# huakunyang/SummerTTS

Hardware: AMD Instinct MI355X
Metric: audio samples/sec (acoustic model + vocoder, phoneme ids -> int16 PCM on host), single_speaker_fast-shaped synthetic blob (higher is better)
Workload: dtype f32 (decoder trunk convs AND the reverse flow's WaveNet convs (wn_flow.hip, one-utterance calls): fp32 operands as 2 fp16 terms = 22-23 of their 24 mantissa bits, 3 fp16 MFMA products per fp32 product, f32 accumulation -- measured error in `parity`, same tolerance as the exact-fp32 leg; batches addi

## Files before the change

### include/summertts_hip.h

```cpp
#ifndef SUMMERTTS_HIP_H_
#define SUMMERTTS_HIP_H_

#include <stdint.h>

#ifdef __cplusplus
extern "C" {
#endif

typedef struct sts_engine sts_engine;

enum {
    STS_OK = 0,
    STS_EINVAL = -1,
    STS_EMODEL = -2,
    STS_EDEVICE = -3,
    STS_ESTATE = -4
};

int sts_create(const float* blob, int64_t blob_bytes, int device, sts_engine** out);
void sts_destroy(sts_engine* e);

int sts_speaker_num(const sts_engine* e);

typedef struct sts_model_info {
// ... 144 lines not shown

enum { STS_DBG_ATTN_BLOCK_MIN_WGS = 1,
       STS_DBG_TAIL_FUSED = 14 ,
       STS_DBG_UPS_ROWPH = 15 ,
       STS_DBG_CHAIN_STREAMS = 13 ,
       STS_DBG_H2P = 11 ,
       STS_DBG_H2P_TILE = 12 ,
       STS_DBG_MEMO_CLEAR = 10 ,
       STS_DBG_PCM_DIRECT = 9 ,
       STS_DBG_DDS_TAIL = 8 ,
       STS_DBG_ATTN_REG = 7 ,
       STS_DBG_LAUNCH_AHEAD = 6 ,
       STS_DBG_FLOW_FUSED = 5  };
enum { STS_DBG_STREAM_RETRY_STEP = 16, STS_DBG_STREAM_DIRECT = 17 };
enum { STS_DBG_POISON = 18 };
int sts_debug_set(sts_engine* e, int key, int value);

typedef struct sts_profile {
    float ms_text_encoder, ms_duration, ms_flow, ms_decoder, ms_total_device;
    float ms_decoder_mfma;
    int32_t decoder_mfma_launches;
    double flops_text_encoder, flops_duration, flops_flow, flops_decoder;
    double flops_decoder_mfma;
    double bytes_decoder_min;
    int64_t frames, samples, phonemes;
    double flops_decoder_mfma_executed;
    double bytes_text_encoder, bytes_duration, bytes_flow;
    float ms_sync_wait_host;
    double flops_decoder_bf16_issued;
    int64_t conv_math_fallbacks;
// ... 115 lines not shown
```

### summertts_amd/csrc/capi.hip

```cpp
#include <stdlib.h>
#include <string.h>

#include <algorithm>
#include <new>
#include <string>
#include <utility>
#include <vector>

#include "engine.hpp"
#include "eq_stream.hpp"
#include "join_stream.hpp"
#include "loud_stream.hpp"

using namespace sts;

struct sts_engine { Engine eng; };

static thread_local std::string g_err;
static int set_err(int code, const std::string& s) { g_err = s; return code; }
#define STS_CAPI_NOT_WHILE_OPEN(e) \
    do { if ((e)->eng.stream_is_open()) return set_err(STS_ESTATE, "a stream is open on this engine (sts_stream_close first)"); } while (0)

extern "C" {

// ... 726 lines not shown
        case STS_DBG_ATTN_BLOCK_MIN_WGS: if (value < 1) return set_err(STS_EINVAL, "threshold must be >= 1"); e->eng.attn_block_min_wgs = value; return STS_OK;
        case STS_DBG_FLOW_FUSED: e->eng.flow_fused = value == 2 || value == 3 ? value : value != 0; return STS_OK;
        case STS_DBG_LAUNCH_AHEAD: if (value < 0 || value > 2) return set_err(STS_EINVAL, "launch_ahead must be 0, 1 or 2"); if ((value == 2) != (e->eng.launch_ahead == 2)) { e->eng.seen_tf_.clear(); e->eng.seen_order_.clear(); } e->eng.launch_ahead = value; return STS_OK;
        case STS_DBG_H2P: e->eng.h2p = value < 0 ? 0 : (value > 4 ? 4 : value); return STS_OK;
        case STS_DBG_H2P_TILE: e->eng.h2p_tile = value; return STS_OK;
        case STS_DBG_CHAIN_STREAMS: e->eng.chain_streams_dbg = value; return STS_OK;
        case STS_DBG_TAIL_FUSED: e->eng.tail_fused = value != 0; return STS_OK;
        case STS_DBG_UPS_ROWPH: e->eng.ups_rowph = value != 0; return STS_OK;
        case STS_DBG_MEMO_CLEAR: e->eng.seen_tf_.clear(); e->eng.seen_order_.clear(); return STS_OK;
        case STS_DBG_ATTN_REG: e->eng.attn_reg = value != 0; return STS_OK;
        case STS_DBG_DDS_TAIL: e->eng.dds_tail = value != 0; return STS_OK;
        case STS_DBG_PCM_DIRECT: e->eng.pcm_direct = value != 0; return STS_OK;
        case STS_DBG_STREAM_RETRY_STEP: e->eng.stream_retry_step = value < 0 ? -1 : value; return STS_OK;
        case STS_DBG_STREAM_DIRECT: e->eng.stream_direct = value != 0; return STS_OK;
        case STS_DBG_POISON: e->eng.poison = (unsigned)value; return STS_OK;
        default: return set_err(STS_EINVAL, "unknown debug key");
    }
}
int sts_set_host_pcm(sts_engine* e, int enable) { if (!e) return set_err(STS_EINVAL, "null engine"); e->eng.host_pcm = enable != 0; return STS_OK; }
int sts_set_profiling(sts_engine* e, int enable) { if (!e) return set_err(STS_EINVAL, "null engine"); e->eng.profiling = enable == 2 ? 2 : (enable != 0 ? 1 : 0); return STS_OK; }

int sts_abi_version(void) { return STS_ABI_VERSION; }

int sts_set_output_rate(sts_engine* e, int32_t rate) {
    if (!e) return set_err(STS_EINVAL, "null engine");
    const int rc = e->eng.set_output_rate(rate);
    return rc == STS_OK ? STS_OK : set_err(rc, e->eng.error());
}
int sts_get_output_rate(const sts_engine* e) {
    if (!e) return set_err(STS_EINVAL, "null engine");
// ... 835 lines not shown
```

### summertts_amd/csrc/conv.hip

```cpp
#include "kernels.hpp"
#include "devmath.hpp"
#include "conv_common.hpp"

namespace sts {

__device__ __forceinline__ float load_in(const ConvArgs& a, const float* xrow, int pos, int in_len, int orig_len) {
    if (pos < 0 || pos >= in_len) return 0.f;
    int src = pos;
    if (a.in_reflect) {
        src = pos - 1;
        if (src < 0) { if (orig_len > 1) src = 1; else return 0.f; }
    }
    float v = xrow[src];
    if (a.in_act) v = v < 0.f ? v * a.in_slope : v;
    return v;
}

#ifndef STS_EXP
#define STS_EXP 0
#endif

#ifndef STS_RA_GROUP
#define STS_RA_GROUP 3
#endif
// ... 769 lines not shown
            }
            static_for<0, 8>([&](auto rc) {
                constexpr int r = decltype(rc)::value;
                const int row = m0 + ((hb + r) & 3) + 8 * ((hb + r) >> 2) + 4 * half;
                const float bv = b2v[r];
                const float ya = acc[0][hb + r] + acc[1][hb + r] + acc[2][hb + r] + bv;
                const float yb = acc[1][hb + r] - acc[2][hb + r] - acc[3][hb + r] + bv;
                const size_t o = (size_t)row * G.ld + opos;
                if (va) a.y[o] = ya + xa[r];
                if (vb) a.y[o + 1] = yb + xb[r];
            });
        });
    }
}

template <int MW, int NW>
__global__ __launch_bounds__(1024) void conv_mfma_splitk_kernel(ConvArgs a, int mtiles) {
    constexpr int G = 4, E = MW * NW * 16;
    constexpr int D = MW * NW == 1 ? 6 : (MW * NW == 2 ? 4 : 3);
    extern __shared__ __attribute__((aligned(16))) float red[];
    const int KS = blockDim.x >> 6;
    const int nsl = a.kslices > 1 ? a.kslices : 1;
    const int b = blockIdx.z / nsl, slice = blockIdx.z - b * nsl;
    const int orig_len = seg_len(a.in_seg, b);
    const int in_len = orig_len + (a.in_reflect ? 1 : 0);
    const int out_len = seg_len(a.out_seg, b);
    const int n_count = a.transposed ? in_len + a.n_extra : out_len;
    const int n0 = blockIdx.x * 32 * NW;
    if (n0 >= n_count) return;
    const int phase = blockIdx.y / mtiles;
    const int m0 = (blockIdx.y - phase * mtiles) * 32 * MW;
    const size_t in_base = (size_t)seg_start(a.in_seg, b), out_base = (size_t)seg_start(a.out_seg, b);
    const int tid = threadIdx.x, lane = tid & 63, wave = tid >> 6;
    const int l31 = lane & 31, half = lane >> 5;
    const float* w = a.w + (size_t)phase * a.ntap * a.Cin_pad * a.Cout_pad;
    bool mvalid[MW];
#pragma unroll
    for (int i = 0; i < MW; i++) mvalid[i] = (m0 + i * 32) < a.Cout_pad;

    f32x16 acc[MW][NW];
#pragma unroll
    for (int i = 0; i < MW; i++)
#pragma unroll
        for (int q = 0; q < NW; q++)
#pragma unroll
            for (int r = 0; r < 16; r++) acc[i][q][r] = 0.f;

    const int gpt = a.Cin_pad / (2 * G);
    const int gall = a.ntap * gpt;
    const int gper = (gall + nsl - 1) / nsl;
    const int gfirst = slice * gper;
    const int ngroups = (STS_EXP & 64) ? gfirst : (gfirst + gper < gall ? gfirst + gper : gall);
    float ra[D][G][MW], rb[D][G][NW];
    const int swave = __builtin_amdgcn_readfirstlane(wave);
    const int sKS = __builtin_amdgcn_readfirstlane(KS);
    const rsrc_t xrs = make_rsrc(a.x + in_base, (unsigned)(((size_t)(a.Cin - 1) * a.x_ld + orig_len) * 4));
    const rsrc_t wrs = make_rsrc(w, (unsigned)((size_t)a.ntap * a.Cin_pad * a.Cout_pad * 4));
    const unsigned ld4 = (unsigned)a.x_ld * 4u;
    const unsigned x_lane = (unsigned)half * ld4;
    const unsigned a_lane = (unsigned)(((size_t)half * a.Cout_pad + m0 + l31) * 4);
    const int lanepos = n0 + l31;
    int lj = (gfirst + swave) / gpt, lc = (gfirst + swave - lj * gpt) * 2 * G;
    const int jstep = sKS / gpt, cstep = (sKS - jstep * gpt) * 2 * G;

    auto load_group = [&](float (&fa)[G][MW], float (&fb)[G][NW]) {
        const int shift = lj * a.tap_step + a.tap_off;
        unsigned off[NW];
#pragma unroll
        for (int q = 0; q < NW; q++) {
            int pos = lanepos + q * 32 + shift;
            bool v = pos >= 0 && pos < in_len;
            if (a.in_reflect) { pos = pos - 1; if (pos < 0) { pos = 1; v = v && orig_len > 1; } }
            off[q] = v ? (unsigned)pos * 4u + x_lane : kOOB;
        }
        const unsigned xs0 = (unsigned)lc * ld4;
        const unsigned ws0 = (unsigned)((((size_t)lj * a.Cin_pad + lc) * a.Cout_pad) * 4);
#pragma unroll
        for (int i = 0; i < G; i++) {
            const bool cv = lc + 2 * i + half < a.Cin;
#pragma unroll
            for (int q = 0; q < NW; q++)
                fb[i][q] = __builtin_bit_cast(float, __builtin_amdgcn_raw_buffer_load_b32(xrs, (int)(cv ? off[q] : kOOB), (int)(xs0 + (unsigned)(2 * i) * ld4), 0));
#pragma unroll
            for (int k = 0; k < MW; k++)
                fa[i][k] = __builtin_bit_cast(float, __builtin_amdgcn_raw_buffer_load_b32(
                    wrs, (int)a_lane, (int)(ws0 + (unsigned)(2 * i) * (unsigned)a.Cout_pad * 4u + (unsigned)k * 128u), 0));
        }
        lj += jstep; lc += cstep;
        if (lc >= a.Cin_pad) { lc -= a.Cin_pad; lj++; }
    };

    int gnext = gfirst + swave;
#pragma unroll
    for (int d = 0; d < D; d++) { if (gnext < ngroups) load_group(ra[d], rb[d]); gnext += sKS; }
    int gcur = gfirst + swave;
    while (gcur < ngroups) {
#pragma unroll
        for (int d = 0; d < D; d++) {
            if (gcur < ngroups) {
#pragma unroll
                for (int i = 0; i < G; i++) {
                    float bq[NW];
#pragma unroll
                    for (int q = 0; q < NW; q++) {
                        float v = rb[d][i][q];
                        if (a.in_act) v = v < 0.f ? v * a.in_slope : v;
                        bq[q] = v;
                    }
#pragma unroll
                    for (int k = 0; k < MW; k++)
#pragma unroll
                        for (int q = 0; q < NW; q++)
                            acc[k][q] = __builtin_amdgcn_mfma_f32_32x32x2f32(ra[d][i][k], bq[q], acc[k][q], 0, 0, 0);
                }
                if (gnext < ngroups) load_group(ra[d], rb[d]);
            }
            gnext += sKS; gcur += sKS;
        }
    }

    static_for<0, MW>([&](auto ic) {
        constexpr int i = decltype(ic)::value;
        static_for<0, NW>([&](auto qc) {
            constexpr int q = decltype(qc)::value;
            static_for<0, 16>([&](auto rc) {
                constexpr int r = decltype(rc)::value;
                red[((size_t)wave * E + (i * NW + q) * 16 + r) * 64 + lane] = acc[i][q][r];
            });
        });
    });
    __syncthreads();
    const int out_off = a.out_off + phase;
    const bool gate = a.epi == EPI_GATE;
    for (int e = wave; e < E; e += KS) {
        const int i = e / (NW * 16);
        const int q = (e >> 4) % NW, r = e & 15;
        if (gate && r >= 8) continue;
        const int n = n0 + q * 32 + l31;
        const int pos = n * a.out_stride + out_off;
        if (n >= n_count || pos < 0 || pos >= out_len) continue;
        const size_t opos = out_base + (size_t)pos;
        const int rowp = m0 + i * 32 + (r & 3) + 8 * (r >> 2) + 4 * half;
        float v = 0.f, v2 = 0.f;
        for (int k = 0; k < KS; k++) {
            v += red[((size_t)k * E + (i * NW + q) * 16 + r) * 64 + lane];
            if (gate) v2 += red[((size_t)k * E + (i * NW + q) * 16 + r + 8) * 64 + lane];
        }
        if (gate) {
            if (!mvalid[i]) continue;
// ... 43 lines not shown
    const long nt = (a.max_n + 127) / 128;
    if (a.Cout_pad % 64 == 0 && nt * (a.Cout_pad / 64) * nphase * a.B >= 512) return 3;
    return 4;
}

template <int MW, int NW, int WM, int WN>
static void launch_mfma(const ConvArgs& a, int nphase, hipStream_t st) {
    constexpr int MT = 32 * MW * WM, NT = 32 * NW * WN;
    const int mt = (a.Cout_pad + MT - 1) / MT;
    const int nx = (a.max_n + NT - 1) / NT, ny = mt * nphase;
    size_t lds = (size_t)2 * CK * (NT + MAX_HALO) * sizeof(float);
    hipLaunchKernelGGL((conv_mfma_kernel<MW, NW, WM, WN>), dim3(mapped_grid(nx, ny, a.B)), dim3(WM * WN * 64), lds, st, a, mt, nx, ny);
}

template <int MW, int NW>
static void launch_splitk(const ConvArgs& a, int nphase, hipStream_t st, bool pinned = false) {
    const int mt = (a.Cout_pad + 32 * MW - 1) / (32 * MW);
    const int nt = (a.max_n + 32 * NW - 1) / (32 * NW);
    const int nsl = a.kslices > 1 ? a.kslices : 1;
    const long steps = ((long)a.ntap * (a.Cin_pad / 8) + nsl - 1) / nsl;
    constexpr int E = MW * NW * 16;
    const bool sparse = !pinned && (long)mt * nt * nphase * a.B * nsl <= 256;
    const int ks_cap = E <= 16 ? 16 : (E <= 32 ? (sparse ? 16 : 8) : 4);
    int ks = 1;
    while (ks < ks_cap && steps / (ks * 2) >= 6 && (pinned || (long)mt * nt * nphase * a.B * nsl * ks * 2 <= 4096)) ks *= 2;
    dim3 grid(nt, mt * nphase, a.B * nsl);
    size_t lds = (size_t)ks * E * 64 * sizeof(float);
    hipLaunchKernelGGL((conv_mfma_splitk_kernel<MW, NW>), grid, dim3(ks * 64), lds, st, a, mt);
}

template <int MW, int NW, int WM, int WN>
static void launch_mfma_group(const ConvGroup& G, hipStream_t st) {
    constexpr int MT = 32 * MW * WM, NT = 32 * NW * WN;
    const ConvArgs& a = G.g[0];
    const int mt = (a.Cout_pad + MT - 1) / MT;
    const int nx = (a.max_n + NT - 1) / NT;
    size_t lds = (size_t)2 * CK * (NT + MAX_HALO) * sizeof(float);
    hipLaunchKernelGGL((conv_mfma_group_kernel<MW, NW, WM, WN>), dim3(mapped_grid(nx, mt, a.B * G.n)), dim3(WM * WN * 64), lds, st, G,
                       mt, a.B, nx, mt);
}

bool resblock_layer_eligible(const ResLayerGroup& G) {
    if (G.n < 1 || G.n > kMaxGroup || (G.C != 32 && G.C != 64 && G.C != 128) || G.max_n <= 0 || G.B <= 0) return false;
// ... 113 lines not shown
            ConvArgs t = G.g[j]; G.g[j] = G.g[j - 1]; G.g[j - 1] = t;
        }
    if (tile != 1 && tile != 3 && tile != 4 && tile != 5) {
        const ConvArgs& a = G.g[0];
        const long nt = (a.max_n + 127) / 128;
        tile = (a.Cout_pad % 64 == 0 && nt * (a.Cout_pad / 64) * a.B * G.n >= 1024) ? 3 : 4;
    }
    switch (tile) {
        case 1: launch_mfma_group<2, 2, 1, 4>(G, st); break;
        case 3: launch_mfma_group<2, 1, 1, 4>(G, st); break;
        case 5: launch_mfma_group<1, 2, 1, 4>(G, st); break;
        default: launch_mfma_group<1, 1, 1, 4>(G, st); break;
    }
}

void conv_mfma(const ConvArgs& a, hipStream_t st, int tile) {
    int nphase = a.transposed ? a.out_stride : 1;
    if (a.max_n <= 0 || a.B <= 0) return;
    const bool pinned = tile == 6 || tile == 7;
    bool splitk = pinned || a.kslices > 1;
    int nw = tile == 7 ? 2 : 1;
    if (a.kslices > 1 && tile != 7) tile = 6;
    if (tile < 0 || tile > 7) {
        tile = pick_tile(a, nphase);
        const TileCfg& t = kTiles[tile];
        const int MT = 32 * t.MW * t.WM, NT = 32 * t.NW * t.WN;
        const long blocks = (long)((a.max_n + NT - 1) / NT) * ((a.Cout_pad + MT - 1) / MT) * nphase * a.B;
        const bool fits32 = (double)a.Cin_pad * (double)a.x_ld * 4.0 < 2.0e9;
        if (blocks < 256 && fits32) { splitk = true; nw = ((a.max_n + 63) / 64) * ((a.Cout_pad + 31) / 32) * nphase * (long)a.B >= 512 ? 2 : 1; }
        else if (a.transposed && blocks < 1024 && (long)a.ntap * (a.Cin_pad / 8) >= 128 && fits32) { splitk = true; nw = 2; }
        else if (a.ntap == 1 && !a.transposed && a.Cin_pad <= 256 && fits32) { splitk = true; nw = 1; }
    }
    if (splitk) {
        if (nw == 2) launch_splitk<1, 2>(a, nphase, st, pinned); else launch_splitk<1, 1>(a, nphase, st, pinned);
        return;
    }
    switch (tile) {
        case 0: launch_mfma<2, 2, 2, 2>(a, nphase, st); break;
        case 1: launch_mfma<2, 2, 1, 4>(a, nphase, st); break;
        case 2: launch_mfma<1, 4, 1, 4>(a, nphase, st); break;
        case 3: launch_mfma<2, 1, 1, 4>(a, nphase, st); break;
        case 4: launch_mfma<1, 1, 1, 4>(a, nphase, st); break;
        default: launch_mfma<1, 2, 1, 4>(a, nphase, st); break;
    }
}

__global__ __launch_bounds__(256) void conv_generic_kernel(ConvArgs a, int rows) {
// ... 184 lines not shown
```

### summertts_amd/csrc/engine.hip

```cpp
#include "run_ctx.hpp"
#include <time.h>
#include "knobs.hpp"
#include "../../include/tts_logger.h"

#include <algorithm>
#include <chrono>
#include <math.h>
#include <new>
#include <stdlib.h>
#include <string.h>
#include <thread>

namespace sts {

#define STS_NOT_WHILE_OPEN(what) \
    do { if (live_) return fail(STS_ESTATE, "a stream is open on this engine (sts_stream_close first): it refuses " what); } while (0)

Engine::~Engine() {
    if (live_) (void)stream_close();
    if (stream) (void)hipStreamSynchronize(stream);
    free_model(model);
    if (arenaT_.base) (void)hipFree(arenaT_.base);
    if (arenaF_.base) (void)hipFree(arenaF_.base);
    if (pinned_) (void)hipHostFree(pinned_);
// ... 135 lines not shown
    if (o.nsum >= 2) { a.xs1 = o.sum1; a.xs2 = o.sum2; a.nsum = o.nsum; }
    const double positions = c.transposed ? (double)lin.total : (double)lout.total;
    const double fl = 2.0 * c.macs_per_out * positions;
    flops_[cur_stage_] += fl;
    {
        const size_t wfl = c.depthwise ? (size_t)c.k * c.Cout : (size_t)c.k * c.Cin * c.Cout;
        double by = 4.0 * ((double)c.Cin * lin.total + (double)c.Cout * lout.total);
        if (o.res || o.epi == EPI_SUB || o.epi == EPI_RESSKIP) by += 4.0 * (double)c.Cout * lout.total;
        bytes_[cur_stage_] += by;
        bytes_w_[cur_stage_] += 4.0 * (double)wfl;
    }
    if (flops) *flops = fl;
    return a;
}

void Engine::conv(const DConv& c, const float* x, const Lvl& lin, float* y, const Lvl& lout, const ConvOpt& o) {
    double fl = 0;
    ConvArgs a = conv_args(c, x, lin, y, lout, o, &fl);
    const bool can_mfma = conv_mode != 1 && conv_mfma_eligible(a);
    const bool use_bf3 = conv_mode == 0 && conv_math != 1 && o.tile < 0 && conv_bf3_eligible(a) &&
                         (in_mfma_region_ || conv_math == 2 || conv_bf3_blocks(a) >= 384);
    if (use_bf3 && c.transposed && ups_rowph && a.epi == EPI_STORE && !a.ubias && (a.math == 1 ? c.wh2r : c.wb3r)) {
        a.wb3 = a.math == 1 ? c.wh2r : c.wb3r;
        a.bias = c.bias ? c.bias_r : nullptr;
        a.Cout = a.Cout_pad = c.Cout_pad * c.stride;
        a.rowph = c.stride;
    }
    if (a.nsum >= 2 && !(use_bf3 ? conv_bf3_takes_sum(a) : (!can_mfma && conv_cout1_takes(a)))) {
        const float* r[3] = {x, o.sum1, o.sum2};
        sum_scale(o.sum_dst, r, a.nsum, o.sum_n, cur_);
        a.x = o.sum_dst; a.xs1 = a.xs2 = nullptr; a.nsum = 0;
    }
    if (use_bf3) {
        if (in_mfma_region_) { mfma_flops_ += fl; bf16_exec_ += products() * fl; mfma_launches_++; }
        static const int bt = exp_int("STS_BF3_TILE", -1);
        conv_bf3(a, cur_, bt);
    } else if (can_mfma) {
        if (in_mfma_region_) { mfma_flops_ += fl; mfma_exec_ += fl; mfma_launches_++; }
        conv_mfma(a, cur_, o.tile >= 0 ? o.tile : (conv_mode >= 2 ? conv_mode - 2 : -1));
    } else {
        if (a.kslices > 1 && a.kslice_stride > 0)
            (void)hipMemsetAsync(a.y + a.kslice_stride, 0, (size_t)(a.kslices - 1) * (size_t)a.kslice_stride * sizeof(float), cur_);
        conv_generic(a, cur_);
    }
}

int Engine::pick_kslices(const DConv& c, const Lvl& lout) const {
    if (conv_mode != 0 || c.depthwise || c.transposed || c.Cin < 32) return 1;
    const long tiles = (long)((lout.max_len + 31) / 32) * (c.Cout_pad / 32) * lout.nb;
    const long groups = (long)c.k * (c.Cin_pad / 8);
    int s = 1;
    while (s < 8 && tiles * (s * 2) <= 256 && groups / (s * 2) >= 24) s *= 2;
    return s;
}

void Engine::ln(const DLn& l, const float* a, const float* b, const float* res, float* y, const Lvl& lv, int pre_relu, int post_gelu, int nb, long b_stride) {
    LnArgs g;
    memset(&g, 0, sizeof(g));
    g.a = a; g.a_ld = lv.ld; g.b = b; g.b_ld = lv.ld; g.res = res; g.res_ld = lv.ld; g.y = y; g.y_ld = lv.ld;
// ... 400 lines not shown
    auto produce_x_and_conv = [&](int l, const DConv& c, float* y) {
        ColProjArgs pj;
        memset(&pj, 0, sizeof(pj));
        pj.x_out = bt.x; pj.x_ld = Ttot; pj.wc = c.wc; pj.bias = c.bias_rows; pj.Cout = c.Cout; pj.npass = (c.Cout + H - 1) / H;
        pj.y = y; pj.y_ld = Ttot; pj.C = H; pj.seg = lvT.seg; pj.B = B; pj.max_len = maxT;
        if (l == 0) { pj.ids = bt.ids; pj.emb = M.emb; pj.vocab = M.vocab; pj.emb_scale = sqrtf((float)M.hidden); }
        else { pj.a = bt.x1; pj.a_ld = Ttot; pj.bp = bt.y; pj.b_ld = Ttot; pj.nb = ffn2_slices; pj.b_stride = (long)H * Ttot;
               pj.gamma = M.ln2[l - 1].g; pj.beta = M.ln2[l - 1].b; }
        const bool ok = !no_colp && conv_mode != 1 && colp_grid && (pj.npass == 1 || colp_blocks >= 24) && c.k == 1 && c.Cin == H && M.emb_size == H && c.wc &&
                        (l == 0 || M.ln2[l - 1].C == H) && col_proj_eligible(pj);
        if (ok) {
            flops_[0] += 2.0 * c.macs_per_out * (double)Ttot;
            bytes_[0] += 4.0 * ((double)H * Ttot * (l == 0 ? 1.0 : 2.0 + ffn2_slices) + (double)c.Cout * Ttot + (double)H * c.Cout);
            col_proj(pj, stream);
            return;
        }
        if (l == 0) embed(bt.ids, M.emb, M.vocab, M.emb_size, sqrtf((float)M.hidden), bt.x, Ttot, (int)Ttot, stream);
        else ln(M.ln2[l - 1], bt.x1, bt.y, nullptr, bt.x, lvT, 0, 0, ffn2_slices, (long)H * Ttot);
        conv(c, bt.x, lvT, y, lvT, ConvOpt());
    };
    for (int l = 0; l < M.n_layers; l++) {
        const DMha& a = M.mha[l];
        produce_x_and_conv(l, a.qkv, bt.qkv);
        AttnArgs at;
        memset(&at, 0, sizeof(at));
        at.q = bt.qkv; at.k = bt.qkv + (size_t)H * Ttot; at.v = bt.qkv + (size_t)2 * H * Ttot; at.o = bt.att; at.ld = Ttot;
        at.relk = a.relk; at.relv = a.relv; at.kc = a.kc; at.px = a.px; at.win = a.win; at.nheads = 2;
        at.seg = lvT.seg; at.B = B; at.max_len = maxT; at.block_min_wgs = attn_block_min_wgs; at.attn_reg = attn_reg;
        attention(at, stream);
        flops_[0] += 2.0 * 2.0 * (double)a.ch * (double)maxT * (double)Ttot;
// ... 1106 lines not shown
```

### summertts_amd/csrc/engine.hpp

```cpp
#pragma once
#include <hip/hip_runtime.h>

#include <deque>
#include <map>
#include <unordered_map>
#include <string>
#include <vector>

#include "../../include/summertts_hip.h"
#include "kernels.hpp"
#include "live_stream.hpp"
#include "model.hpp"

namespace sts {

struct Arena {
    char* base = nullptr; size_t cap = 0, used = 0; bool measuring = false;
    void* alloc(size_t bytes) {
        size_t a = (used + 255) & ~(size_t)255;
        used = a + bytes;
        if (measuring) return nullptr;
        return base + a;
    }
    template <typename T> T* get(size_t count) { return (T*)alloc(count * sizeof(T)); }
// ... 96 lines not shown
    int pcm_direct = 1;
    int dds_tail = 1;
    int attn_reg = 1;
    int attn_block_min_wgs = 96;
    int launch_ahead = 1;
    long ahead_misses = 0;
    static constexpr size_t kMemoEntries = 1024;
    std::unordered_map<unsigned long long, long> seen_tf_; std::deque<unsigned long long> seen_order_;
    bool polite_wait = false;
    struct WaitEst { double us = 0.0; long phonemes = 0; };
    WaitEst wait_est_[2][24];
    void nap_before_wait(int which, long phonemes);
    void note_wait(int which, long phonemes, double waited_us, bool was_ready_at_wake);
    int final_sync(long phonemes);
    int ups_rowph = 1;
    int tail_fused = 1;
    int chain_streams_dbg = -1;
    int h2p = 1;
    int h2p_tile = -1;
    int flow_fused = 1;
    int n_cus = 0;
    int stream_retry_step = -1;
    int stream_direct = 0;
    unsigned poison = 0;
    int64_t poison_bytes_ = 0;
    hipStream_t stream = nullptr;

private:
    int fail(int code, const std::string& msg) { err_ = msg; return code; }
    bool ensure(Arena& a, size_t bytes);
    bool ensure_pinned(size_t bytes);
    void poison_arena(const Arena& a);
    void poison_host16(void* p, size_t samples);
    void poison_host32(void* p, size_t words);
    ConvArgs conv_args(const DConv& c, const float* x, const Lvl& lin, float* y, const Lvl& lout, const ConvOpt& o, double* flops);
    void conv(const DConv& c, const float* x, const Lvl& lin, float* y, const Lvl& lout, const ConvOpt& o);
    void ln(const DLn& l, const float* a, const float* b, const float* res, float* y, const Lvl& lv, int pre_relu, int post_gelu, int nb = 1, long b_stride = 0);
    int pick_kslices(const DConv& c, const Lvl& lout) const;
    struct SplineTail { const DConv* proj; float filter_sqrt; const float* r0; const float* r1; float* o0; float* o1; };
    float* dds(const DDds& d, float* h, float* t1, float* t2, const Lvl& lv, const DConv* pre = nullptr, const float* pre_in = nullptr,
               const float* pre_res = nullptr, const SplineTail* tail = nullptr, bool* tail_done = nullptr);
    int run_any_math(int B, const int32_t* const* ids, const int32_t* n, const int32_t* sid, const float* ls, const StreamSpec* ss);
    struct RunCtx;
    struct ResStage;
    int run_setup(RunCtx& c);
    int run_text_encoder(RunCtx& c);
    int run_durations(RunCtx& c);
    int run_frame_workspace(RunCtx& c);
    int run_flow(RunCtx& c);
    int run_decode(RunCtx& c, int nw, long Wtot, int maxW, int zoff0, int wlen0);
    int decode_end(RunCtx& c, const float* wave, const WinGeom& win, long Wtot, int maxW);
// ... 58 lines not shown
```

### summertts_amd/csrc/kernels.hpp

```cpp
#pragma once
#include <hip/hip_runtime.h>
#include <stdint.h>

#include <vector>

#include "../../include/summertts_hip.h"

namespace sts {

struct SegView {
    const int* off;
    const int* len;
    int scale;
    int extra;
    int ioff, ilen;
};

enum Epilogue : int {
    EPI_STORE = 0,
    EPI_RESADD = 1,
    EPI_SUB = 3,
    EPI_GATE = 4,
    EPI_RESSKIP = 5,
    EPI_TANH_PCM = 6,
// ... 108 lines not shown
    const float* b_res; const float* b_m;
    unsigned* ovf;
};
struct FlowFinishArgs {
    SegView seg; int B, max_len; int half;
    const float* src; long src_ld; float* dst; long dst_ld;
    const float* macc; int n; long macc_stride;
};
bool flow_layer_shape_ok(int H, int half, int k, int dil, int n_layers);
int flow_layer_groups(int H);
void flow_layer(const FlowLayerArgs& a, hipStream_t st, int nt = 32);
void flow_finish(const FlowFinishArgs& a, hipStream_t st);

bool conv_mfma_eligible(const ConvArgs& a);
void conv_mfma(const ConvArgs& a, hipStream_t st, int tile = -1);
constexpr int kMaxGroup = 4;
struct ConvGroup { ConvArgs g[kMaxGroup]; int n; };
struct ResLayerArgs {
    const float* x; float* y;
    const float *w1, *b1, *w2, *b2;
    int k1, dil1, k2;
    const float *wu1, *wu2;
    const void *wb1, *wb2;
    float ws1, ws2;
};
struct ResLayerGroup {
    ResLayerArgs g[kMaxGroup];
    int n, C; long ld; float slope;
    SegView seg; int B; int max_n;
    int math; unsigned* ovf;
// ... 237 lines not shown
```

### summertts_amd/csrc/misc_kernels.hip

```cpp
#include "kernels.hpp"
#include "devmath.hpp"
#include "knobs.hpp"
#include "noise.hpp"
#include <stdlib.h>
#include <string.h>

namespace sts {

__device__ __forceinline__ int seg_start(const SegView& s, int b) { return (s.off ? s.off[b] : s.ioff) * s.scale + b * s.extra; }
__device__ __forceinline__ int seg_len(const SegView& s, int b) { return (s.off ? s.len[b] : s.ilen) * s.scale + s.extra; }

__device__ __forceinline__ float wave_sum(float v) {
#pragma unroll
    for (int o = 32; o > 0; o >>= 1) v += __shfl_xor(v, o, 64);
    return v;
}

__global__ void embed_kernel(const int* ids, const float* emb, int vocab, int H, float scale, float* x, long ld, int total) {
    long i = (long)blockIdx.x * blockDim.x + threadIdx.x;
    if (i >= (long)H * total) return;
    int h = (int)(i / total), pos = (int)(i - (long)h * total);
    int id = ids[pos];
    if (id < 0 || id >= vocab) id = 0;
    x[(size_t)h * ld + pos] = emb[(size_t)h * vocab + id] * scale;
}
void embed(const int* ids, const float* emb, int vocab, int H, float scale, float* x, long ld, int total, hipStream_t st) {
    long n = (long)H * total;
    if (n <= 0) return;
    hipLaunchKernelGGL(embed_kernel, dim3((unsigned)((n + 255) / 256)), dim3(256), 0, st, ids, emb, vocab, H, scale, x, ld, total);
}

constexpr int LN_G = 32;
__device__ __forceinline__ float ln_input(const LnArgs& a, int c, size_t p, int pos, int len) {
    float v;
    if (a.dw_w) {
        v = a.dw_b ? a.dw_b[c] : 0.f;
        const float* row = a.a + (size_t)c * a.a_ld + (p - pos);
        int j = 0;
        for (; j + 2 < a.dw_k; j += 3) {
            const int q0 = pos + j * a.dw_dil - a.dw_pad, q1 = q0 + a.dw_dil, q2 = q1 + a.dw_dil;
            const float w0 = a.dw_w[(size_t)j * a.dw_ld + c], w1 = a.dw_w[(size_t)(j + 1) * a.dw_ld + c], w2 = a.dw_w[(size_t)(j + 2) * a.dw_ld + c];
            const float x0 = row[q0 >= 0 && q0 < len ? q0 : pos], x1 = row[q1 >= 0 && q1 < len ? q1 : pos], x2 = row[q2 >= 0 && q2 < len ? q2 : pos];
            v += w0 * ((q0 >= 0 && q0 < len) ? x0 : 0.f);
            v += w1 * ((q1 >= 0 && q1 < len) ? x1 : 0.f);
            v += w2 * ((q2 >= 0 && q2 < len) ? x2 : 0.f);
        }
        for (; j < a.dw_k; j++) {
            const int q = pos + j * a.dw_dil - a.dw_pad;
            if (q >= 0 && q < len) v += a.dw_w[(size_t)j * a.dw_ld + c] * row[q];
        }
    } else {
        v = a.a[(size_t)c * a.a_ld + p];
    }
    if (a.b) {
        if (a.nb > 1) {
            float pb[8];
#pragma unroll
            for (int q = 0; q < 8; q++) pb[q] = q < a.nb ? a.b[(size_t)q * a.b_stride + (size_t)c * a.b_ld + p] : 0.f;
            float bs = pb[0];
#pragma unroll
            for (int q = 1; q < 8; q++) bs += pb[q];
            v += bs;
        } else {
            v += a.b[(size_t)c * a.b_ld + p];
        }
    }
    if (a.pre_relu && v < 0.f) v = 0.f;
    return v;
}
__global__ __launch_bounds__(1024) void layer_norm_kernel(LnArgs a) {
    __shared__ float rs[LN_G][33], rq[LN_G][33];
    const int b = blockIdx.y;
    const int len = seg_len(a.seg, b);
    const int tx = threadIdx.x & 31, cy = threadIdx.x >> 5;
    const int pos = blockIdx.x * 32 + tx;
    const bool live = pos < len;
    const size_t p = (size_t)seg_start(a.seg, b) + (live ? pos : 0);
    constexpr int MAXV = 8;
    float vals[MAXV], gam[MAXV], bet[MAXV], rsd[MAXV];
    float s = 0.f, sq = 0.f;
    if (live) {
#pragma unroll
        for (int u = 0; u < MAXV; u++) {
            const int c = cy + u * LN_G;
            if (c < a.C) { gam[u] = a.gamma[c]; bet[u] = a.beta[c]; rsd[u] = a.res ? a.res[(size_t)c * a.res_ld + p] : 0.f; }
        }
#pragma unroll
        for (int u = 0; u < MAXV; u++) {
            const int c = cy + u * LN_G;
            if (c < a.C) { const float v = ln_input(a, c, p, pos, len); vals[u] = v; s += v; sq += v * v; }
        }
        for (int c = cy + MAXV * LN_G; c < a.C; c += LN_G) { const float v = ln_input(a, c, p, pos, len); s += v; sq += v * v; }
    }
    rs[cy][tx] = s; rq[cy][tx] = sq;
    __syncthreads();
    if (!live) return;
    s = 0.f; sq = 0.f;
#pragma unroll
    for (int k = 0; k < LN_G; k++) { s += rs[k][tx]; sq += rq[k][tx]; }
    const float mean = s / (float)a.C;
    const float scale = (float)(1. / (float)a.C);
    const float var = sq * scale - mean * mean;
    const float den = (float)sqrt((double)var + 1e-05);
    auto finish = [&](int c, float v) {
        float o = ((v - mean) / den) * a.gamma[c] + a.beta[c];
        if (a.post_gelu) o = gelu_ref(o);
        if (a.res) o = a.res[(size_t)c * a.res_ld + p] + o;
        a.y[(size_t)c * a.y_ld + p] = o;
    };
#pragma unroll
    for (int u = 0; u < MAXV; u++) {
        const int c = cy + u * LN_G;
        if (c < a.C) {
            float o = ((vals[u] - mean) / den) * gam[u] + bet[u];
            if (a.post_gelu) o = gelu_ref(o);
            if (a.res) o = rsd[u] + o;
            a.y[(size_t)c * a.y_ld + p] = o;
        }
    }
    for (int c = cy + MAXV * LN_G; c < a.C; c += LN_G) finish(c, ln_input(a, c, p, pos, len));
}
void layer_norm(const LnArgs& a, hipStream_t st) {
    if (a.max_len <= 0 || a.B <= 0) return;
    hipLaunchKernelGGL(layer_norm_kernel, dim3((a.max_len + 31) / 32, a.B), dim3(1024), 0, st, a);
}

__global__ __launch_bounds__(256) void attention_kernel(AttnArgs a) {
    extern __shared__ __attribute__((aligned(16))) float sm[];
    const int b = blockIdx.z, h = blockIdx.y, i = blockIdx.x;
// ... 882 lines not shown
```

### summertts_amd/engine.py

```python
from __future__ import annotations

import ctypes as C
import os
import subprocess
from typing import Dict, List, Optional, Sequence

import numpy as np

_HERE = os.path.dirname(os.path.abspath(__file__))
LIB_PATH = os.environ.get("SUMMERTTS_HIP_LIB") or os.path.join(_HERE, "lib", "libsummertts_hip.so")
CSRC = os.path.join(_HERE, "csrc")


def build_library(verbose: bool = False) -> str:
    subprocess.run(["make", "-C", CSRC, "-j8"], check=True, stdout=None if verbose else subprocess.DEVNULL)
    return LIB_PATH


class ModelInfo(C.Structure):
    _fields_ = [("is_multi_speaker", C.c_int32), ("lang_type", C.c_int32), ("dur_pred_type", C.c_int32),
                ("dec_type", C.c_int32), ("vocab", C.c_int32), ("hidden", C.c_int32), ("inter_channels", C.c_int32),
                ("speaker_num", C.c_int32), ("gin_channels", C.c_int32), ("samples_per_frame", C.c_int32),
                ("sample_rate", C.c_int32), ("blob_floats_consumed", C.c_int64)]

# ... 1026 lines not shown
        out = np.zeros(n, LIMITER_DTYPE)
        if n:
            rc = self.lib.sts_get_limiter(self.h, out.ctypes.data, n)
            if rc < 0:
                _check(self.lib, rc)
        return out

    def set_conv_math(self, mode):
        m = {"bf16x3": 0, "f32": 1, "bf16x3_all": 2, "f16x2": 3}.get(mode, mode)
        _check(self.lib, self.lib.sts_set_conv_math(self.h, int(m)))

    def set_conv_mode(self, mode: int):
        _check(self.lib, self.lib.sts_set_conv_mode(self.h, mode))

    def debug_set(self, key: str, value: int):
        _check(self.lib, self.lib.sts_debug_set(self.h, {"attn_block_min_wgs": 1, "flow_fused": 5, "launch_ahead": 6, "attn_reg": 7, "dds_tail": 8, "pcm_direct": 9, "memo_clear": 10, "h2p": 11, "h2p_tile": 12, "chain_streams": 13, "tail_fused": 14, "ups_rowph": 15, "stream_retry_step": 16, "stream_direct": 17, "poison": 18}[key], int(value)))

    def set_profiling(self, on):
        _check(self.lib, self.lib.sts_set_profiling(self.h, 2 if on == 2 else (1 if on else 0)))

    def profile(self) -> dict:
        p = Profile()
        _check(self.lib, self.lib.sts_get_profile_ex(self.h, C.byref(p), C.sizeof(p)))
        return p.as_dict()

    def tap(self, name: str) -> np.ndarray:
        ptr = C.POINTER(C.c_float)()
        ch, ln = C.c_int32(), C.c_int64()
        _check(self.lib, self.lib.sts_get_tap(self.h, name.encode(), C.byref(ptr), C.byref(ch), C.byref(ln)))
        a = np.ctypeslib.as_array(ptr, shape=(ch.value, ln.value)).copy()
        self.lib.sts_free(ptr)
# ... 430 lines not shown
```

Baseline: 67.75 million.

## Fold embedding and layer-norm prologue into text-encoder 1x1 MFMA split-K conv

Adds a prologue mode to the split-K MFMA conv kernel. Extra waves gather the embedding lookup (first layer) or the residual-sum plus LayerNorm (later layers) into LDS, and the 1x1 text-encoder projection then reads its B operand from LDS instead of launching a separate embed or LN kernel. Block 0 along y also writes the normalized activations back to global memory for the residual path. It applies only when the grid fits within the CU count, and the goal is to remove a kernel launch and a global round trip per layer. The cost is that every M-tile block recomputes the LN/embedding, uses more LDS, and needs extra syncs, so occupancy may drop.

Result: no change. 67.92 million (median of 5 runs) (+0.3%).

```diff
diff --git a/include/summertts_hip.h b/include/summertts_hip.h
--- a/include/summertts_hip.h
+++ b/include/summertts_hip.h
@@ -182,6 +182,7 @@
        STS_DBG_FLOW_FUSED = 5  };
 enum { STS_DBG_STREAM_RETRY_STEP = 16, STS_DBG_STREAM_DIRECT = 17 };
 enum { STS_DBG_POISON = 18 };
+enum { STS_DBG_TE_FOLD = 19 };
 int sts_debug_set(sts_engine* e, int key, int value);
 
 typedef struct sts_profile {
diff --git a/summertts_amd/csrc/capi.hip b/summertts_amd/csrc/capi.hip
--- a/summertts_amd/csrc/capi.hip
+++ b/summertts_amd/csrc/capi.hip
@@ -764,6 +764,7 @@
         case STS_DBG_STREAM_RETRY_STEP: e->eng.stream_retry_step = value < 0 ? -1 : value; return STS_OK;
         case STS_DBG_STREAM_DIRECT: e->eng.stream_direct = value != 0; return STS_OK;
         case STS_DBG_POISON: e->eng.poison = (unsigned)value; return STS_OK;
+        case STS_DBG_TE_FOLD: e->eng.te_fold = value != 0; return STS_OK;
         default: return set_err(STS_EINVAL, "unknown debug key");
     }
 }
diff --git a/summertts_amd/csrc/conv.hip b/summertts_amd/csrc/conv.hip
--- a/summertts_amd/csrc/conv.hip
+++ b/summertts_amd/csrc/conv.hip
@@ -1,6 +1,7 @@
 #include "kernels.hpp"
 #include "devmath.hpp"
 #include "conv_common.hpp"
+#include "ln_dev.hpp"
 
 namespace sts {
 
@@ -807,12 +808,14 @@
     }
 }
 
-template <int MW, int NW>
-__global__ __launch_bounds__(1024) void conv_mfma_splitk_kernel(ConvArgs a, int mtiles) {
+template <int PRO> struct SplitkPro { ConvProArgs p; int ks; };
+template <> struct SplitkPro<0> {};
+template <int MW, int NW, int PRO = 0>
+__global__ __launch_bounds__(1024) void conv_mfma_splitk_kernel(ConvArgs a, int mtiles, SplitkPro<PRO> pro) {
     constexpr int G = 4, E = MW * NW * 16;
     constexpr int D = MW * NW == 1 ? 6 : (MW * NW == 2 ? 4 : 3);
     extern __shared__ __attribute__((aligned(16))) float red[];
-    const int KS = blockDim.x >> 6;
+    const int KS = [&] { if constexpr (PRO != 0) return pro.ks; else return (int)(blockDim.x >> 6); }();
     const int nsl = a.kslices > 1 ? a.kslices : 1;
     const int b = blockIdx.z / nsl, slice = blockIdx.z - b * nsl;
     const int orig_len = seg_len(a.in_seg, b);
@@ -843,7 +846,8 @@
     const int gall = a.ntap * gpt;
     const int gper = (gall + nsl - 1) / nsl;
     const int gfirst = slice * gper;
-    const int ngroups = (STS_EXP & 64) ? gfirst : (gfirst + gper < gall ? gfirst + gper : gall);
+    const int ngroups = ((STS_EXP & 64) || (PRO != 0 && __builtin_amdgcn_readfirstlane((int)threadIdx.x >> 6) >= KS))
+                            ? gfirst : (gfirst + gper < gall ? gfirst + gper : gall);
     float ra[D][G][MW], rb[D][G][NW];
     const int swave = __builtin_amdgcn_readfirstlane(wave);
     const int sKS = __builtin_amdgcn_readfirstlane(KS);
@@ -856,7 +860,29 @@
     int lj = (gfirst + swave) / gpt, lc = (gfirst + swave - lj * gpt) * 2 * G;
     const int jstep = sKS / gpt, cstep = (sKS - jstep * gpt) * 2 * G;
 
+    constexpr int XW = 32 * NW;
+    float* const xs = red + (size_t)KS * E * 64;
+    auto load_a0 = [&](float (&fa)[G][MW], int c) {
+        const unsigned ws0 = (unsigned)(((size_t)c * a.Cout_pad) * 4);
+#pragma unroll
+        for (int i = 0; i < G; i++)
+#pragma unroll
+            for (int k = 0; k < MW; k++)
+                fa[i][k] = __builtin_bit_cast(float, __builtin_amdgcn_raw_buffer_load_b32(
+                    wrs, (int)a_lane, (int)(ws0 + (unsigned)(2 * i) * (unsigned)a.Cout_pad * 4u + (unsigned)k * 128u), 0));
+    };
+    auto load_b0 = [&](float (&fb)[G][NW], int c) {
+#pragma unroll
+        for (int i = 0; i < G; i++)
+#pragma unroll
+            for (int q = 0; q < NW; q++) fb[i][q] = xs[(c + 2 * i + half) * XW + q * 32 + l31];
+    };
     auto load_group = [&](float (&fa)[G][MW], float (&fb)[G][NW]) {
+        if constexpr (PRO != 0) {
+            load_b0(fb, lc); load_a0(fa, lc);
+            lc += cstep;
+            return;
+        }
         const int shift = lj * a.tap_step + a.tap_off;
         unsigned off[NW];
 #pragma unroll
@@ -884,8 +910,102 @@
     };
 
     int gnext = gfirst + swave;
-#pragma unroll
-    for (int d = 0; d < D; d++) { if (gnext < ngroups) load_group(ra[d], rb[d]); gnext += sKS; }
+    if constexpr (PRO == 0) {
+#pragma unroll
+        for (int d = 0; d < D; d++) { if (gnext < ngroups) load_group(ra[d], rb[d]); gnext += sKS; }
+    } else {
+#pragma unroll
+        for (int d = 0; d < D; d++) { if (gnext + d * sKS < ngroups) load_a0(ra[d], lc + d * cstep); }
+        const ConvProArgs& p = pro.p;
+        const int C = a.Cin;
+        const int tx = tid % XW, cg = tid / XW, ncg = (int)blockDim.x / XW;
+        const int pos = n0 + tx;
+        const bool live = pos < orig_len;
+        const size_t gp = in_base + (size_t)(live ? pos : 0);
+        const bool wr = live && blockIdx.y == 0;
+        if constexpr (PRO == 2) {
+            int id = p.ids[gp];
+            if (id < 0 || id >= p.vocab) id = 0;
+            constexpr int EB = 8;
+            for (int c0 = cg; c0 < C; c0 += EB * ncg) {
+                float e[EB];
+#pragma unroll
+                for (int k = 0; k < EB; k++) { const int c = c0 + k * ncg; e[k] = p.emb[(size_t)(c < C ? c : cg) * p.vocab + id]; }
+#pragma unroll
+                for (int k = 0; k < EB; k++) {
+                    const int c = c0 + k * ncg;
+                    if (c < C) {
+                        const float v = live ? e[k] * p.emb_scale : 0.f;
+                        xs[c * XW + tx] = v;
+                        if (wr) p.x_out[(size_t)c * p.x_ld + gp] = v;
+                    }
+                }
+            }
+        } else {
+            float* const st_s = xs + (size_t)C * XW;
+            float* const st_q = st_s + LN_G * XW;
+            float* const gb = st_q + LN_G * XW;
+            for (int c = tid; c < C; c += (int)blockDim.x) { gb[c] = p.gamma[c]; gb[C + c] = p.beta[c]; }
+            auto gather = [&](auto nbc) {
+                constexpr int NBC = decltype(nbc)::value;
+                constexpr int EB = 8;
+                for (int c0 = cg; c0 < C; c0 += EB * ncg) {
+                    float va[EB], pb[EB][8];
+#pragma unroll
+                    for (int k = 0; k < EB; k++) {
+                        const int c = c0 + k * ncg;
+                        const size_t o = (size_t)(c < C ? c : cg);
+                        va[k] = p.a[o * p.a_ld + gp];
+#pragma unroll
+                        for (int q = 0; q < 8; q++)
+                            pb[k][q] = q < NBC ? p.bp[(size_t)(q < p.nb ? q : 0) * p.b_stride + o * p.b_ld + gp] : 0.f;
+                    }
+#pragma unroll
+                    for (int k = 0; k < EB; k++) {
+                        const int c = c0 + k * ncg;
+#pragma unroll
+                        for (int q = 1; q < NBC; q++) pb[k][q] = q < p.nb ? pb[k][q] : 0.f;
+                        const float v = p.nb > 1 ? va[k] + ln_sum8(pb[k]) : va[k] + pb[k][0];
+                        if (c < C) xs[c * XW + tx] = live ? v : 0.f;
+                    }
+                }
+            };
+            if (p.nb > 4) gather(std::integral_constant<int, 8>{});
+            else if (p.nb > 2) gather(std::integral_constant<int, 4>{});
+            else if (p.nb == 2) gather(std::integral_constant<int, 2>{});
+            else if (p.nb == 1) gather(std::integral_constant<int, 1>{});
+            else {
+                for (int c = cg; c < C; c += ncg) { const float v = p.a[(size_t)c * p.a_ld + gp]; xs[c * XW + tx] = live ? v : 0.f; }
+            }
+            __syncthreads();
+            for (int cy = cg; cy < LN_G; cy += ncg) {
+                float s = 0.f, sq = 0.f;
+#pragma unroll
+                for (int u = 0; u < 8; u++) {
+                    const int c = cy + u * LN_G;
+                    if (c < C) ln_acc(xs[c * XW + tx], s, sq);
+                }
+                st_s[cy * XW + tx] = s; st_q[cy * XW + tx] = sq;
+            }
+            __syncthreads();
+            if (live) {
+                float s = 0.f, sq = 0.f;
+#pragma unroll
+                for (int k = 0; k < LN_G; k++) { s += st_s[k * XW + tx]; sq += st_q[k * XW + tx]; }
+                float mean, den;
+                ln_stats(s, sq, C, mean, den);
+#pragma unroll 4
+                for (int c = cg; c < C; c += ncg) {
+                    const float o = ln_norm(xs[c * XW + tx], mean, den, gb[c], gb[C + c]);
+                    xs[c * XW + tx] = o;
+                    if (wr) p.x_out[(size_t)c * p.x_ld + gp] = o;
+                }
+            }
+        }
+        __syncthreads();
+#pragma unroll
+        for (int d = 0; d < D; d++) { if (gnext < ngroups) { load_b0(rb[d], lc); lc += cstep; } gnext += sKS; }
+    }
     int gcur = gfirst + swave;
     while (gcur < ngroups) {
 #pragma unroll
@@ -912,7 +1032,7 @@
         }
     }
 
-    static_for<0, MW>([&](auto ic) {
+    if (PRO == 0 || wave < KS) static_for<0, MW>([&](auto ic) {
         constexpr int i = decltype(ic)::value;
         static_for<0, NW>([&](auto qc) {
             constexpr int q = decltype(qc)::value;
@@ -925,7 +1045,8 @@
     __syncthreads();
     const int out_off = a.out_off + phase;
     const bool gate = a.epi == EPI_GATE;
-    for (int e = wave; e < E; e += KS) {
+    const int nwaves = PRO != 0 ? (int)(blockDim.x >> 6) : KS;
+    for (int e = wave; e < E; e += nwaves) {
         const int i = e / (NW * 16);
         const int q = (e >> 4) % NW, r = e & 15;
         if (gate && r >= 8) continue;
@@ -999,7 +1120,7 @@
 }
 
 template <int MW, int NW>
-static void launch_splitk(const ConvArgs& a, int nphase, hipStream_t st, bool pinned = false) {
+static int splitk_waves(const ConvArgs& a, int nphase, bool pinned) {
     const int mt = (a.Cout_pad + 32 * MW - 1) / (32 * MW);
     const int nt = (a.max_n + 32 * NW - 1) / (32 * NW);
     const int nsl = a.kslices > 1 ? a.kslices : 1;
@@ -1009,9 +1130,18 @@
     const int ks_cap = E <= 16 ? 16 : (E <= 32 ? (sparse ? 16 : 8) : 4);
     int ks = 1;
     while (ks < ks_cap && steps / (ks * 2) >= 6 && (pinned || (long)mt * nt * nphase * a.B * nsl * ks * 2 <= 4096)) ks *= 2;
+    return ks;
+}
+template <int MW, int NW>
+static void launch_splitk(const ConvArgs& a, int nphase, hipStream_t st, bool pinned = false) {
+    const int mt = (a.Cout_pad + 32 * MW - 1) / (32 * MW);
+    const int nt = (a.max_n + 32 * NW - 1) / (32 * NW);
+    const int nsl = a.kslices > 1 ? a.kslices : 1;
+    constexpr int E = MW * NW * 16;
+    const int ks = splitk_waves<MW, NW>(a, nphase, pinned);
     dim3 grid(nt, mt * nphase, a.B * nsl);
     size_t lds = (size_t)ks * E * 64 * sizeof(float);
-    hipLaunchKernelGGL((conv_mfma_splitk_kernel<MW, NW>), grid, dim3(ks * 64), lds, st, a, mt);
+    hipLaunchKernelGGL((conv_mfma_splitk_kernel<MW, NW>), grid, dim3(ks * 64), lds, st, a, mt, SplitkPro<0>{});
 }
 
 template <int MW, int NW, int WM, int WN>
@@ -1155,6 +1285,43 @@
     }
 }
 
+static bool auto_splitk(const ConvArgs& a, int nphase, int* tile, int* nw) {
+    *tile = pick_tile(a, nphase);
+    const TileCfg& t = kTiles[*tile];
+    const int MT = 32 * t.MW * t.WM, NT = 32 * t.NW * t.WN;
+    const long blocks = (long)((a.max_n + NT - 1) / NT) * ((a.Cout_pad + MT - 1) / MT) * nphase * a.B;
+    const bool fits32 = (double)a.Cin_pad * (double)a.x_ld * 4.0 < 2.0e9;
+    if (blocks < 256 && fits32) { *nw = ((a.max_n + 63) / 64) * ((a.Cout_pad + 31) / 32) * nphase * (long)a.B >= 512 ? 2 : 1; return true; }
+    if (a.transposed && blocks < 1024 && (long)a.ntap * (a.Cin_pad / 8) >= 128 && fits32) { *nw = 2; return true; }
+    if (a.ntap == 1 && !a.transposed && a.Cin_pad <= 256 && fits32) { *nw = 1; return true; }
+    return false;
+}
+
+bool conv_mfma_staged(const ConvArgs& a, const ConvProArgs& p, hipStream_t st) {
+    if (a.max_n <= 0 || a.B <= 0 || !conv_mfma_eligible(a)) return false;
+    if (a.ntap != 1 || a.tap_off != 0 || a.transposed || a.in_reflect || a.kslices > 1 || a.in_act || a.nsum >= 2) return false;
+    if (a.out_stride != 1 || a.out_off != 0 || a.Cin != a.Cin_pad || a.Cin > 256 || !p.x_out) return false;
+    const SegView &si = a.in_seg, &so = a.out_seg;
+    if (si.off != so.off || si.len != so.len || si.scale != so.scale || si.extra != so.extra || si.ioff != so.ioff || si.ilen != so.ilen) return false;
+    if (p.mode == 1) { if (!p.a || !p.gamma || !p.beta || p.nb < 0 || p.nb > 8 || (p.nb > 0 && !p.bp)) return false; }
+    else if (p.mode == 2) { if (!p.ids || !p.emb || p.vocab <= 0) return false; }
+    else return false;
+    int tile, nw;
+    if (!auto_splitk(a, 1, &tile, &nw) || nw != 1) return false;
+    const int ks = splitk_waves<1, 1>(a, 1, false);
+    if (ks >= a.Cin_pad / 8) return false;
+    const int C = a.Cin;
+    int pw = C > 64 ? 16 : 8;
+    if (pw < ks) pw = ks;
+    const size_t lds = ((size_t)ks * 16 * 64 + (size_t)C * 32 + (p.mode == 1 ? (size_t)2 * LN_G * 32 + 2 * (size_t)C : 0)) * sizeof(float);
+    if (lds > 64 * 1024) return false;
+    const int mt = (a.Cout_pad + 31) / 32, nt = (a.max_n + 31) / 32;
+    const dim3 grid(nt, mt, a.B);
+    if (p.mode == 1) hipLaunchKernelGGL((conv_mfma_splitk_kernel<1, 1, 1>), grid, dim3(pw * 64), lds, st, a, mt, SplitkPro<1>{p, ks});
+    else hipLaunchKernelGGL((conv_mfma_splitk_kernel<1, 1, 2>), grid, dim3(pw * 64), lds, st, a, mt, SplitkPro<2>{p, ks});
+    return true;
+}
+
 void conv_mfma(const ConvArgs& a, hipStream_t st, int tile) {
     int nphase = a.transposed ? a.out_stride : 1;
     if (a.max_n <= 0 || a.B <= 0) return;
@@ -1162,16 +1329,7 @@
     bool splitk = pinned || a.kslices > 1;
     int nw = tile == 7 ? 2 : 1;
     if (a.kslices > 1 && tile != 7) tile = 6;
-    if (tile < 0 || tile > 7) {
-        tile = pick_tile(a, nphase);
-        const TileCfg& t = kTiles[tile];
-        const int MT = 32 * t.MW * t.WM, NT = 32 * t.NW * t.WN;
-        const long blocks = (long)((a.max_n + NT - 1) / NT) * ((a.Cout_pad + MT - 1) / MT) * nphase * a.B;
-        const bool fits32 = (double)a.Cin_pad * (double)a.x_ld * 4.0 < 2.0e9;
-        if (blocks < 256 && fits32) { splitk = true; nw = ((a.max_n + 63) / 64) * ((a.Cout_pad + 31) / 32) * nphase * (long)a.B >= 512 ? 2 : 1; }
-        else if (a.transposed && blocks < 1024 && (long)a.ntap * (a.Cin_pad / 8) >= 128 && fits32) { splitk = true; nw = 2; }
-        else if (a.ntap == 1 && !a.transposed && a.Cin_pad <= 256 && fits32) { splitk = true; nw = 1; }
-    }
+    if (tile < 0 || tile > 7) splitk = auto_splitk(a, nphase, &tile, &nw);
     if (splitk) {
         if (nw == 2) launch_splitk<1, 2>(a, nphase, st, pinned); else launch_splitk<1, 1>(a, nphase, st, pinned);
         return;
diff --git a/summertts_amd/csrc/engine.hip b/summertts_amd/csrc/engine.hip
--- a/summertts_amd/csrc/engine.hip
+++ b/summertts_amd/csrc/engine.hip
@@ -173,12 +173,21 @@
     return a;
 }
 
-void Engine::conv(const DConv& c, const float* x, const Lvl& lin, float* y, const Lvl& lout, const ConvOpt& o) {
+bool Engine::conv(const DConv& c, const float* x, const Lvl& lin, float* y, const Lvl& lout, const ConvOpt& o, const ConvProArgs* pro) {
     double fl = 0;
+    const double fl0 = flops_[cur_stage_], by0 = bytes_[cur_stage_], bw0 = bytes_w_[cur_stage_];
     ConvArgs a = conv_args(c, x, lin, y, lout, o, &fl);
     const bool can_mfma = conv_mode != 1 && conv_mfma_eligible(a);
     const bool use_bf3 = conv_mode == 0 && conv_math != 1 && o.tile < 0 && conv_bf3_eligible(a) &&
                          (in_mfma_region_ || conv_math == 2 || conv_bf3_blocks(a) >= 384);
+    if (pro) {
+        if (conv_mode == 0 && o.tile < 0 && can_mfma && !use_bf3 && a.nsum < 2 && conv_mfma_staged(a, *pro, cur_)) {
+            if (in_mfma_region_) { mfma_flops_ += fl; mfma_exec_ += fl; mfma_launches_++; }
+            return true;
+        }
+        flops_[cur_stage_] = fl0; bytes_[cur_stage_] = by0; bytes_w_[cur_stage_] = bw0;
+        return false;
+    }
     if (use_bf3 && c.transposed && ups_rowph && a.epi == EPI_STORE && !a.ubias && (a.math == 1 ? c.wh2r : c.wb3r)) {
         a.wb3 = a.math == 1 ? c.wh2r : c.wb3r;
         a.bias = c.bias ? c.bias_r : nullptr;
@@ -202,6 +211,7 @@
             (void)hipMemsetAsync(a.y + a.kslice_stride, 0, (size_t)(a.kslices - 1) * (size_t)a.kslice_stride * sizeof(float), cur_);
         conv_generic(a, cur_);
     }
+    return false;
 }
 
 int Engine::pick_kslices(const DConv& c, const Lvl& lout) const {
@@ -632,6 +642,19 @@
             bytes_[0] += 4.0 * ((double)H * Ttot * (l == 0 ? 1.0 : 2.0 + ffn2_slices) + (double)c.Cout * Ttot + (double)H * c.Cout);
             col_proj(pj, stream);
             return;
+        }
+        const long te_wgs = (long)((maxT + 31) / 32) * ((c.Cout_pad + 31) / 32) * B;
+        if (te_fold && te_wgs <= n_cus && c.k == 1 && c.Cin == H && (l == 0 ? M.emb_size == H : M.ln2[l - 1].C == H)) {
+            ConvProArgs pr;
+            memset(&pr, 0, sizeof(pr));
+            pr.x_out = bt.x; pr.x_ld = Ttot;
+            if (l == 0) { pr.mode = 2; pr.ids = bt.ids; pr.emb = M.emb; pr.vocab = M.vocab; pr.emb_scale = sqrtf((float)M.hidden); }
+            else { pr.mode = 1; pr.a = bt.x1; pr.a_ld = Ttot; pr.bp = bt.y; pr.b_ld = Ttot; pr.nb = ffn2_slices; pr.b_stride = (long)H * Ttot;
+                   pr.gamma = M.ln2[l - 1].g; pr.beta = M.ln2[l - 1].b; }
+            if (conv(c, bt.x, lvT, y, lvT, ConvOpt(), &pr)) {
+                bytes_[0] += l == 0 ? 4.0 * (double)Ttot : 4.0 * ((double)H * Ttot * (1.0 + ffn2_slices) + 2.0 * H);
+                return;
+            }
         }
         if (l == 0) embed(bt.ids, M.emb, M.vocab, M.emb_size, sqrtf((float)M.hidden), bt.x, Ttot, (int)Ttot, stream);
         else ln(M.ln2[l - 1], bt.x1, bt.y, nullptr, bt.x, lvT, 0, 0, ffn2_slices, (long)H * Ttot);
diff --git a/summertts_amd/csrc/engine.hpp b/summertts_amd/csrc/engine.hpp
--- a/summertts_amd/csrc/engine.hpp
+++ b/summertts_amd/csrc/engine.hpp
@@ -134,6 +134,7 @@
     void note_wait(int which, long phonemes, double waited_us, bool was_ready_at_wake);
     int final_sync(long phonemes);
     int ups_rowph = 1;
+    int te_fold = 1;
     int tail_fused = 1;
     int chain_streams_dbg = -1;
     int h2p = 1;
@@ -154,7 +155,7 @@
     void poison_host16(void* p, size_t samples);
     void poison_host32(void* p, size_t words);
     ConvArgs conv_args(const DConv& c, const float* x, const Lvl& lin, float* y, const Lvl& lout, const ConvOpt& o, double* flops);
-    void conv(const DConv& c, const float* x, const Lvl& lin, float* y, const Lvl& lout, const ConvOpt& o);
+    bool conv(const DConv& c, const float* x, const Lvl& lin, float* y, const Lvl& lout, const ConvOpt& o, const ConvProArgs* pro = nullptr);
     void ln(const DLn& l, const float* a, const float* b, const float* res, float* y, const Lvl& lv, int pre_relu, int post_gelu, int nb = 1, long b_stride = 0);
     int pick_kslices(const DConv& c, const Lvl& lout) const;
     struct SplineTail { const DConv* proj; float filter_sqrt; const float* r0; const float* r1; float* o0; float* o1; };
diff --git a/summertts_amd/csrc/kernels.hpp b/summertts_amd/csrc/kernels.hpp
--- a/summertts_amd/csrc/kernels.hpp
+++ b/summertts_amd/csrc/kernels.hpp
@@ -146,6 +146,14 @@
 
 bool conv_mfma_eligible(const ConvArgs& a);
 void conv_mfma(const ConvArgs& a, hipStream_t st, int tile = -1);
+struct ConvProArgs {
+    int mode;
+    const float* a; long a_ld; const float* bp; long b_ld; int nb; long b_stride;
+    const float* gamma; const float* beta;
+    const int* ids; const float* emb; int vocab; float emb_scale;
+    float* x_out; long x_ld;
+};
+bool conv_mfma_staged(const ConvArgs& a, const ConvProArgs& p, hipStream_t st);
 constexpr int kMaxGroup = 4;
 struct ConvGroup { ConvArgs g[kMaxGroup]; int n; };
 struct ResLayerArgs {
diff --git a/summertts_amd/csrc/ln_dev.hpp b/summertts_amd/csrc/ln_dev.hpp
--- /dev/null
+++ b/summertts_amd/csrc/ln_dev.hpp
@@ -0,0 +1,23 @@
+#pragma once
+#include <hip/hip_runtime.h>
+
+namespace sts {
+
+constexpr int LN_G = 32;
+
+__device__ __forceinline__ void ln_acc(float v, float& s, float& sq) { s += v; sq += v * v; }
+__device__ __forceinline__ void ln_stats(float s, float sq, int C, float& mean, float& den) {
+    mean = s / (float)C;
+    const float scale = (float)(1. / (float)C);
+    const float var = sq * scale - mean * mean;
+    den = (float)sqrt((double)var + 1e-05);
+}
+__device__ __forceinline__ float ln_norm(float v, float mean, float den, float gamma, float beta) { return ((v - mean) / den) * gamma + beta; }
+__device__ __forceinline__ float ln_sum8(const float (&pb)[8]) {
+    float bs = pb[0];
+#pragma unroll
+    for (int q = 1; q < 8; q++) bs += pb[q];
+    return bs;
+}
+
+}
diff --git a/summertts_amd/csrc/misc_kernels.hip b/summertts_amd/csrc/misc_kernels.hip
--- a/summertts_amd/csrc/misc_kernels.hip
+++ b/summertts_amd/csrc/misc_kernels.hip
@@ -1,6 +1,7 @@
 #include "kernels.hpp"
 #include "devmath.hpp"
 #include "knobs.hpp"
+#include "ln_dev.hpp"
 #include "noise.hpp"
 #include <stdlib.h>
 #include <string.h>
@@ -30,7 +31,6 @@
     hipLaunchKernelGGL(embed_kernel, dim3((unsigned)((n + 255) / 256)), dim3(256), 0, st, ids, emb, vocab, H, scale, x, ld, total);
 }
 
-constexpr int LN_G = 32;
 __device__ __forceinline__ float ln_input(const LnArgs& a, int c, size_t p, int pos, int len) {
     float v;
     if (a.dw_w) {
@@ -57,10 +57,7 @@
             float pb[8];
 #pragma unroll
             for (int q = 0; q < 8; q++) pb[q] = q < a.nb ? a.b[(size_t)q * a.b_stride + (size_t)c * a.b_ld + p] : 0.f;
-            float bs = pb[0];
-#pragma unroll
-            for (int q = 1; q < 8; q++) bs += pb[q];
-            v += bs;
+            v += ln_sum8(pb);
         } else {
             v += a.b[(size_t)c * a.b_ld + p];
         }
@@ -88,9 +85,9 @@
 #pragma unroll
         for (int u = 0; u < MAXV; u++) {
             const int c = cy + u * LN_G;
-            if (c < a.C) { const float v = ln_input(a, c, p, pos, len); vals[u] = v; s += v; sq += v * v; }
-        }
-        for (int c = cy + MAXV * LN_G; c < a.C; c += LN_G) { const float v = ln_input(a, c, p, pos, len); s += v; sq += v * v; }
+            if (c < a.C) { const float v = ln_input(a, c, p, pos, len); vals[u] = v; ln_acc(v, s, sq); }
+        }
+        for (int c = cy + MAXV * LN_G; c < a.C; c += LN_G) { const float v = ln_input(a, c, p, pos, len); ln_acc(v, s, sq); }
     }
     rs[cy][tx] = s; rq[cy][tx] = sq;
     __syncthreads();
@@ -98,12 +95,10 @@
     s = 0.f; sq = 0.f;
 #pragma unroll
     for (int k = 0; k < LN_G; k++) { s += rs[k][tx]; sq += rq[k][tx]; }
-    const float mean = s / (float)a.C;
-    const float scale = (float)(1. / (float)a.C);
-    const float var = sq * scale - mean * mean;
-    const float den = (float)sqrt((double)var + 1e-05);
+    float mean, den;
+    ln_stats(s, sq, a.C, mean, den);
     auto finish = [&](int c, float v) {
-        float o = ((v - mean) / den) * a.gamma[c] + a.beta[c];
+        float o = ln_norm(v, mean, den, a.gamma[c], a.beta[c]);
         if (a.post_gelu) o = gelu_ref(o);
         if (a.res) o = a.res[(size_t)c * a.res_ld + p] + o;
         a.y[(size_t)c * a.y_ld + p] = o;
@@ -112,7 +107,7 @@
     for (int u = 0; u < MAXV; u++) {
         const int c = cy + u * LN_G;
         if (c < a.C) {
-            float o = ((vals[u] - mean) / den) * gam[u] + bet[u];
+            float o = ln_norm(vals[u], mean, den, gam[u], bet[u]);
             if (a.post_gelu) o = gelu_ref(o);
             if (a.res) o = rsd[u] + o;
             a.y[(size_t)c * a.y_ld + p] = o;
diff --git a/summertts_amd/engine.py b/summertts_amd/engine.py
--- a/summertts_amd/engine.py
+++ b/summertts_amd/engine.py
@@ -1064,7 +1064,7 @@
         _check(self.lib, self.lib.sts_set_conv_mode(self.h, mode))
 
     def debug_set(self, key: str, value: int):
-        _check(self.lib, self.lib.sts_debug_set(self.h, {"attn_block_min_wgs": 1, "flow_fused": 5, "launch_ahead": 6, "attn_reg": 7, "dds_tail": 8, "pcm_direct": 9, "memo_clear": 10, "h2p": 11, "h2p_tile": 12, "chain_streams": 13, "tail_fused": 14, "ups_rowph": 15, "stream_retry_step": 16, "stream_direct": 17, "poison": 18}[key], int(value)))
+        _check(self.lib, self.lib.sts_debug_set(self.h, {"attn_block_min_wgs": 1, "flow_fused": 5, "launch_ahead": 6, "attn_reg": 7, "dds_tail": 8, "pcm_direct": 9, "memo_clear": 10, "h2p": 11, "h2p_tile": 12, "chain_streams": 13, "tail_fused": 14, "ups_rowph": 15, "stream_retry_step": 16, "stream_direct": 17, "poison": 18, "te_fold": 19}[key], int(value)))
 
     def set_profiling(self, on):
         _check(self.lib, self.lib.sts_set_profiling(self.h, 2 if on == 2 else (1 if on else 0)))
```
